# hahnicity/deepards

Measured on AMD Instinct MI355X. Metric: breath-sequences/sec (train step) cnn_linear nb20 seq224, higher is better.
Workload: dtype f32; 1 GPU; cnn_linear+resnet18, synthetic (B=64 per GPU, 20, 1, 224) fp32 train step (BASELINE configs[1]); backbone=resnet18, batch_per_gpu=64, global_batch=64, batch_rule=--batch 64 per rank (weak scaling: the global batch grows with the ranks), n_sub_batches=20, seq_len=224, optimizer=sgd-nesterov+clamp, parallelism=dp1, hipgraph=True

## Files before the change

### deepards_amd/csrc/conv_gemm.hip

```cpp
#include "common.h"
#include <algorithm>
#include <utility>
#include <vector>

#ifndef WGRAD_GLOAD_AT
#define WGRAD_GLOAD_AT 8
#endif
#ifndef GLOAD_AT
#define GLOAD_AT 3
#endif

struct ConvGemmArgs {
  const float* x;
  const float* w;
  const float* x2;
  const float* w2;
  int tap_split;
  float* y;
  int M, Lsrc, ldx, C;
  int Ldst, ldy, N;
  int dst_stride, dst_off, src_stride;
  int ntaps, so0, so1, so2, wt0, wt1, wt2;
  int accumulate;
  FastDiv divLm;
// ... 260 lines not shown
  const int lr = tid >> 3, lq = tid & 7;
  const int Lm = (int)a.divLm.d;

  const int m_a = m_blk + lr;
  const bool a_ok = m_a < a.M;
  const uint32_t row_a = fdiv((uint32_t)(a_ok ? m_a : 0), a.divLm);
  const int a_rowoff = (int)row_a * a.Lsrc;
  const int a_j = ((a_ok ? m_a : 0) - (int)row_a * Lm) * a.src_stride;

  const int kc = a.C >> 6;
  const int nk = a.ntaps * kc;
  f32x4 ra[2], rb[4];
  auto gload = [&](int it) {
    const int t = it / kc;
    const int c0 = (it - t * kc) << 6;
    const int so = t == 0 ? a.so0 : (t == 1 ? a.so1 : a.so2);
    const int wt = t == 0 ? a.wt0 : (t == 1 ? a.wt1 : a.wt2);
    const int ls = a_j + so;
    const bool ok = a_ok && ls >= 0 && ls < a.Lsrc;
    const float* src = (t < a.tap_split ? a.x : a.x2) + (size_t)(a_rowoff + (ok ? ls : 0)) * a.ldx + c0 + lq * 4;
#pragma unroll
    for (int h = 0; h < 2; ++h) {
      f32x4 v = {0.f, 0.f, 0.f, 0.f};
      if (ok) v = *reinterpret_cast<const f32x4*>(src + 32 * h);
      ra[h] = v;
    }
    const float* wtp = (t < a.tap_split ? a.w : a.w2) + (size_t)wt * a.N * a.C + c0 + lq * 4;
#pragma unroll
    for (int p = 0; p < 2; ++p)
#pragma unroll
      for (int h = 0; h < 2; ++h)
        rb[2 * p + h] = *reinterpret_cast<const f32x4*>(wtp + (size_t)(n_blk + lr + 32 * p) * a.C + 32 * h);
  };

  f32x16 acc;
#pragma unroll
  for (int r = 0; r < 16; ++r) acc[r] = 0.f;
  const int frow = lane & 31, fh = lane >> 5;
  gload(0);
  for (int it = 0; it < nk; ++it) {
    __syncthreads();
#pragma unroll
    for (int h = 0; h < 2; ++h) *reinterpret_cast<f32x4*>(&As[(h * 32 + lr) * PITCH + lq * 4]) = ra[h];
#pragma unroll
    for (int p = 0; p < 2; ++p)
#pragma unroll
      for (int h = 0; h < 2; ++h)
        *reinterpret_cast<f32x4*>(&Bs[(h * 64 + lr + 32 * p) * PITCH + lq * 4]) = rb[2 * p + h];
    __syncthreads();
#pragma unroll
    for (int c8 = 0; c8 < 4; ++c8) {
      if (c8 == 3) {
        __builtin_amdgcn_sched_barrier(0);
        if (it + 1 < nk) gload(it + 1);
        __builtin_amdgcn_sched_barrier(0);
      }
      const f32x4 af = *reinterpret_cast<const f32x4*>(&As[(ks * 32 + frow) * PITCH + c8 * 8 + fh * 4]);
      const f32x4 bf = *reinterpret_cast<const f32x4*>(&Bs[(ks * 64 + wn * 32 + frow) * PITCH + c8 * 8 + fh * 4]);
#pragma unroll
      for (int e = 0; e < 4; ++e) acc = __builtin_amdgcn_mfma_f32_32x32x2f32(af[e], bf[e], acc, 0, 0, 0);
    }
  }

  __syncthreads();
  float* red = lds;
  if (ks == 1) {
#pragma unroll
    for (int r = 0; r < 16; ++r) red[(wn * 16 + r) * 64 + lane] = acc[r];
  }
  __syncthreads();
  if (ks == 1) return;
#pragma unroll
  for (int r = 0; r < 16; ++r) acc[r] += red[(wn * 16 + r) * 64 + lane];

  size_t off[16];
  bool ok[16];
#pragma unroll
  for (int r = 0; r < 16; ++r) {
    const int m = m_blk + (r & 3) + 8 * (r >> 2) + 4 * fh;
    ok[r] = m < a.M;
    const uint32_t row = fdiv((uint32_t)(ok[r] ? m : 0), a.divLm);
    const int jj = (ok[r] ? m : 0) - (int)row * Lm;
    off[r] = ((size_t)row * a.Ldst + (size_t)(jj * a.dst_stride + a.dst_off)) * a.ldy;
  }
  const int n = n_blk + wn * 32 + frow;
  if (a.accumulate) {
    float old[16];
#pragma unroll
    for (int r = 0; r < 16; ++r) old[r] = ok[r] ? a.y[off[r] + n] : 0.f;
#pragma unroll
    for (int r = 0; r < 16; ++r)
      if (ok[r]) a.y[off[r] + n] = acc[r] + old[r];
  } else {
#pragma unroll
    for (int r = 0; r < 16; ++r)
      if (ok[r]) a.y[off[r] + n] = acc[r];
  }
}

template <bool HALO>
__global__ __launch_bounds__(256) void conv_gemm_tailed_kernel(ConvGemmArgs a, int nmini, int nmini_pad, int full) {
  __shared__ float lds[HALO ? HALO_LDS_FLOATS : TAIL_LDS_FLOATS];
  if ((int)blockIdx.x < nmini_pad) {
    if ((int)blockIdx.x < nmini) conv_tail_body(a, full + ((int)blockIdx.x >> 1), blockIdx.x & 1, lds);
    return;
  }
  if (HALO) conv3_halo_body(a, blockIdx.x - nmini_pad, full, lds);
  else conv_gemm_body<1, 1, 2, 2>(a, xcd_chunked(blockIdx.x - nmini_pad, full), lds);
}

static int g_use_tail = 1;

template <bool HALO>
static int launch_conv64(const ConvGemmArgs& a, hipStream_t s) {
  const int tiles = ((a.M + 63) / 64) * (a.N / 64);
  const int R = tiles % 256;
  if (g_use_tail && a.C % 64 == 0 && tiles > 256 && R >= 1 && R <= 128) {
    const int full = tiles - R, nmini = 2 * R, nmini_pad = (nmini + 7) / 8 * 8;
    hipLaunchKernelGGL((conv_gemm_tailed_kernel<HALO>), dim3(nmini_pad + full), dim3(256), 0, s, a, nmini, nmini_pad, full);
  } else if (HALO) {
    hipLaunchKernelGGL(conv3_halo_kernel, dim3(tiles), dim3(256), 0, s, a);
  } else {
    hipLaunchKernelGGL((conv_gemm_kernel<1, 1, 2, 2>), dim3(tiles), dim3(256), 0, s, a);
  }
  DA_CHECK_LAUNCH();
  return DA_OK;
}

static double balance(long blocks) {
  double per = (double)blocks / 256.0;
  double mx = (double)((blocks + 255) / 256);
  return per / mx;
}

struct ConvGemmTable {
  ConvGemmArgs d[4];
  int first_block[5];
  int n;
  int tail_first;
};

__global__ __launch_bounds__(256) void conv_gemm_multi_kernel(ConvGemmTable t, int nmini, int nmini_pad) {
  __shared__ float lds[TAIL_LDS_FLOATS];
  if ((int)blockIdx.x < nmini_pad) {
    if ((int)blockIdx.x < nmini) conv_tail_body(t.d[t.n - 1], t.tail_first + ((int)blockIdx.x >> 1), blockIdx.x & 1, lds);
    return;
  }
  const int g = blockIdx.x - nmini_pad;
  int i = 0;
  while (i + 1 < t.n && g >= t.first_block[i + 1]) ++i;
  conv_gemm_body<1, 1, 2, 2>(t.d[i], xcd_chunked(g - t.first_block[i], t.first_block[i + 1] - t.first_block[i]), lds);
}

static int launch_conv_multi(const ConvGemmArgs* a, int n, hipStream_t s) {
  ConvGemmTable t;
  int tiles = 0, last = 0;
  bool tail_ok = g_use_tail != 0;
  for (int i = 0; i < n; ++i) {
    t.d[i] = a[i];
    t.first_block[i] = tiles;
    last = ((a[i].M + 63) / 64) * (a[i].N / 64);
    tiles += last;
    tail_ok = tail_ok && a[i].C % 64 == 0;
  }
  t.n = n;
  if (tiles == 0) return DA_OK;
  const int R = tiles % 256;
  int nmini = 0;
  if (tail_ok && tiles > 256 && R >= 1 && R <= 128 && R < last) nmini = 2 * R;
  t.first_block[n] = tiles - nmini / 2;
  t.tail_first = last - nmini / 2;
  const int nmini_pad = (nmini + 7) / 8 * 8;
  hipLaunchKernelGGL(conv_gemm_multi_kernel, dim3(nmini_pad + t.first_block[n]), dim3(256), 0, s, t, nmini, nmini_pad);
  DA_CHECK_LAUNCH();
  return DA_OK;
}

static int conv_gemm_dispatch(const ConvGemmArgs& a, hipStream_t s) {
  if (a.M <= 0) return DA_OK;
  if (a.C % 32 || a.N % 32 || a.ldx % 4 || a.ntaps < 1 || a.ntaps > 3) return DA_EINVAL;
  if ((uint64_t)a.M * (uint64_t)a.divLm.d >= 0xffffffffull) return DA_EINVAL;
  if (a.C >= 128 && a.ntaps == 3 && a.src_stride == 1 && a.dst_stride == 1 && a.dst_off == 0 && a.N % 64 == 0 &&
      a.Lsrc == (int)a.divLm.d && a.Ldst == (int)a.divLm.d && a.so0 >= -1 && a.so0 <= 1 && a.so1 >= -1 && a.so1 <= 1 &&
      a.so2 >= -1 && a.so2 <= 1) {
    return launch_conv64<true>(a, s);
  }
  struct Cand { int id, bm, bn; double eff; };
  static const Cand cands[] = {{1, 128, 128, 1.00}, {2, 64, 128, 0.99}, {3, 128, 64, 0.97}, {4, 64, 64, 0.93},
                               {5, 128, 32, 0.85}, {6, 32, 128, 0.85}};
  int best = 0;
  double best_score = -1.0;
  for (const Cand& c : cands) {
    if (a.N % c.bn) continue;
    long blocks = (long)((a.M + c.bm - 1) / c.bm) * (a.N / c.bn);
    double score = c.eff * balance(blocks);
    if (score > best_score) {
      best_score = score;
      best = c.id;
    }
  }
  switch (best) {
    case 1: return launch_conv_gemm<2, 2, 2, 2>(a, s);
    case 2: return launch_conv_gemm<1, 2, 2, 2>(a, s);
    case 3: return launch_conv_gemm<1, 2, 4, 1>(a, s);
    case 4: return launch_conv64<false>(a, s);
    case 5: return launch_conv_gemm<1, 1, 4, 1>(a, s);
    case 6: return launch_conv_gemm<1, 1, 1, 4>(a, s);
    default: return DA_EINVAL;
  }
}

struct Conv1x1BnArgs {
  const float* x;
  const float* w;
  float* y;
  int M, ldx, C, ldy, N, W, Wn, ldstat;
  float* mean;
  float* invstd;
  const float* gamma;
  const float* beta;
  FastDiv divWn;
  const float* pend;
  int pend_c0, pend_nc, pend_Wu, pend_tiles;
  float eps;
  float* out_part;
};

template <int POOL, int OSTATS = 0>
__global__ __launch_bounds__(256) void conv1x1_bn_kernel(Conv1x1BnArgs a) {
  extern __shared__ __attribute__((aligned(16))) float lds[];
  constexpr int PITCH = 36;
  float* As = lds;
  float* Bs = lds + 64 * PITCH;
  float* scs = lds + 128 * PITCH;
  float* shs = scs + 2 * a.C;
  const int tid = threadIdx.x, lane = tid & 63, wave = tid >> 6;
  const int wm = wave >> 1, wn = wave & 1;
  const int ntn = a.N >> 6;
  const int lin = xcd_chunked(blockIdx.x, gridDim.x);
  const int m_blk = (lin / ntn) * 64, n_blk = (lin % ntn) * 64;
  const int lr = tid >> 3, lq = tid & 7;
  const int w0 = (int)fdiv((uint32_t)m_blk, a.divWn);

  int a_off[2], a_ws[2];
  bool a_ok[2];
#pragma unroll
  for (int p = 0; p < 2; ++p) {
    const int m = m_blk + lr + 32 * p;
    a_ok[p] = m < a.M;
    const int mm = a_ok[p] ? m : 0;
    a_ws[p] = ((int)fdiv((uint32_t)mm, a.divWn) - w0) * a.C + lq * 4;
    a_off[p] = (POOL ? 2 * mm : mm) * a.ldx + lq * 4;
  }
  const float* wb = a.w + (size_t)(n_blk + lr) * a.C + lq * 4;

  const int kc = a.C >> 5;
  f32x4 ra[2][POOL + 1], rb[2];
  auto gload = [&](int it) {
    const int c0 = it << 5;
#pragma unroll
    for (int p = 0; p < 2; ++p)
#pragma unroll
      for (int h = 0; h <= POOL; ++h) {
        f32x4 v = {0.f, 0.f, 0.f, 0.f};
        if (a_ok[p]) v = *reinterpret_cast<const f32x4*>(a.x + a_off[p] + h * a.ldx + c0);
        ra[p][h] = v;
      }
#pragma unroll
    for (int p = 0; p < 2; ++p) rb[p] = *reinterpret_cast<const f32x4*>(wb + (size_t)(32 * p) * a.C + c0);
  };

  f32x16 acc;
#pragma unroll
  for (int r = 0; r < 16; ++r) acc[r] = 0.f;
  gload(0);
  for (int i = tid; i < 2 * a.C; i += 256) {
    const int ws = i >= a.C ? 1 : 0, c = i - ws * a.C, w = w0 + ws;
    float sc = 0.f, sh = 0.f;
    if (w < a.W) {
      float mu, is;
      if (c >= a.pend_c0) {
        merge_stat_records(a.pend, a.pend_tiles, a.pend_nc, a.pend_Wu, w, c - a.pend_c0, a.eps, mu, is);
        const int mw = w * a.Wn;
        if (n_blk == 0 && mw >= m_blk && mw < m_blk + 64) {
          a.mean[(size_t)w * a.ldstat + c] = mu;
          a.invstd[(size_t)w * a.ldstat + c] = is;
        }
      } else {
        mu = a.mean[(size_t)w * a.ldstat + c];
        is = a.invstd[(size_t)w * a.ldstat + c];
      }
      bn_scale_shift(mu, is, a.gamma[c], a.beta[c], sc, sh);
    }
    scs[i] = sc;
    shs[i] = sh;
  }
  const int frow = lane & 31, fh = lane >> 5;
  for (int it = 0; it < kc; ++it) {
    __syncthreads();
    const int c0 = it << 5;
#pragma unroll
    for (int p = 0; p < 2; ++p) {
      const f32x4 sc = *reinterpret_cast<const f32x4*>(&scs[a_ws[p] + c0]);
      const f32x4 sh = *reinterpret_cast<const f32x4*>(&shs[a_ws[p] + c0]);
      f32x4 h;
#pragma unroll
      for (int e = 0; e < 4; ++e) {
// ... 444 lines not shown
}


static void wgrad_fill_args(WgradArgs& a, const da_wgrad_job& j, const WgradPlan& pl) {
  a.dy = j.dy; a.x = j.x; a.slab = j.workspace;
  a.M = j.rows * j.Lm; a.Ldy = j.Ldy; a.lddy = j.lddy; a.N = j.N;
  a.Lx = j.Lx; a.ldx = j.ldx; a.C = j.C;
  a.dy_stride = j.dy_stride; a.dy_off = j.dy_off; a.src_stride = j.src_stride;
  a.ntaps = j.ntaps;
  a.so0 = j.src_off[0]; a.so1 = j.ntaps > 1 ? j.src_off[1] : 0; a.so2 = j.ntaps > 2 ? j.src_off[2] : 0;
  a.kchunk = pl.kchunk;
  a.divLm = make_fastdiv((uint32_t)j.Lm);
  a.xform = j.xform; a.dy_half = j.dy_half; a.ldstat = j.ldstat;
  a.kind = 0;
  a.mean = j.mean; a.invstd = j.invstd; a.gamma = j.gamma; a.beta = j.beta;
  a.divWn = make_fastdiv((uint32_t)(j.Wn > 0 ? j.Wn : 1));
}

template <int TM, int TN, int WGM, int WGN, int XF = 0>
static int launch_wgrad_group(const da_wgrad_job* jobs, const WgradPlan* plan, int n, int tn, int tc, hipStream_t s, WgradChain* chain) {
  constexpr int BM = TM * WGM * 32, BN = TN * WGN * 32;
  WgradTable t;
  int cnt = 0, blocks = 0;
  auto flush = [&]() -> int {
    if (!cnt) return DA_OK;
    t.n = cnt;
    t.first_block[cnt] = blocks;
    WgradPreTable pre = wgrad_chain_take(chain);
    hipLaunchKernelGGL((conv_wgrad_multi_kernel<TM, TN, WGM, WGN, XF>), dim3(wgrad_pre_grid(pre, blocks, true)), dim3(256), 0, s, t, pre);
    DA_CHECK_LAUNCH();
    cnt = 0;
    blocks = 0;
    return DA_OK;
  };
  std::vector<std::pair<int, int>> order;
  for (int i = 0; i < n; ++i) {
    if (jobs[i].winograd) continue;
    if ((XF != 0) != (jobs[i].xform != 0 || jobs[i].dy_half != 0)) continue;
    if (plan[i].tn == tn && plan[i].tc == tc) order.push_back({-plan[i].kchunk, i});
  }
  std::stable_sort(order.begin(), order.end());
  for (const auto& o : order) {
    const da_wgrad_job& j = jobs[o.second];
    const WgradPlan& pl = plan[o.second];
    wgrad_fill_args(t.d[cnt], j, pl);
    t.first_block[cnt] = blocks;
    blocks += (j.N / BM) * (j.C / BN) * j.ntaps * pl.splits;
    wgrad_chain_offer(chain, o.second, j, pl.splits);
    if (++cnt == WGRAD_TABLE_MAX) {
      int rc = flush();
      if (rc) return rc;
    }
  }
  return flush();
}

static int g_wgrad_any = 1;

template <int XF>
static int launch_wgrad_any(const da_wgrad_job* jobs, const WgradPlan* plan, int n, hipStream_t s, WgradChain* chain) {
  WgradAnyTable t;
  int cnt = 0, blocks = 0;
  auto flush = [&]() -> int {
    if (!cnt) return DA_OK;
    t.n = cnt;
    t.first_block[cnt] = blocks;
    WgradPreTable pre = wgrad_chain_take(chain);
    hipLaunchKernelGGL((conv_wgrad_any_kernel<XF>), dim3(wgrad_pre_grid(pre, blocks, true)), dim3(256), 0, s, t, pre);
    DA_CHECK_LAUNCH();
    cnt = 0;
    blocks = 0;
    return DA_OK;
  };
  std::vector<std::pair<long, int>> order;
  for (int i = 0; i < n; ++i) {
    if (jobs[i].winograd) continue;
    if ((XF != 0) != (jobs[i].xform != 0 || jobs[i].dy_half != 0)) continue;
    const WgradPlan& pl = plan[i];
    if (pl.tn == 128 && pl.tc == 128) continue;
    order.push_back({-(long)pl.kchunk * (pl.tn * pl.tc / 4096), i});
  }
  std::stable_sort(order.begin(), order.end());
  for (const auto& o : order) {
    const da_wgrad_job& j = jobs[o.second];
    const WgradPlan& pl = plan[o.second];
    wgrad_fill_args(t.d[cnt], j, pl);
    t.d[cnt].kind = pl.tn == 128 ? (pl.tc == 64 ? 0 : 3) : (pl.tn == 64 ? (pl.tc == 128 ? 1 : 2) : 4);
    t.first_block[cnt] = blocks;
    blocks += (j.N / pl.tn) * (j.C / pl.tc) * j.ntaps * pl.splits;
    wgrad_chain_offer(chain, o.second, j, pl.splits);
    if (++cnt == WGRAD_TABLE_MAX) {
      int rc = flush();
      if (rc) return rc;
    }
  }
  return flush();
}

int wgrad_plan_jobs(const da_wgrad_job* jobs, int n, int chained, WgradPlan* plan) {
  if (n < 0 || (n && (!jobs || !plan))) return DA_EINVAL;
  int n_xf = 0;
  for (int i = 0; i < n; ++i) {
    const da_wgrad_job& j = jobs[i];
    if (!j.dy || !j.x || j.ntaps < 1 || j.ntaps > 3 || j.C % 32 || j.N % 32 || j.lddy % 4 || j.ldx % 4 ||
        (j.winograd == 49 && (j.lddy != j.N || j.ldx != j.C)))
      return DA_EINVAL;
    if ((uint64_t)j.rows * j.Lm * (uint64_t)j.Lm >= 0xffffffffull) return DA_EINVAL;
    if (j.winograd != 0 && j.winograd != 1 && j.winograd != 6 && j.winograd != 16 && j.winograd != 49) return DA_EINVAL;
    if ((j.xform || j.dy_half) && (j.winograd || j.src_stride != 1 || j.dy_stride != 1 || j.dy_off || j.Lm != j.Lx ||
                                   (j.dy_half && j.ntaps != 1)))
      return DA_EINVAL;
    if (j.dy_half && !j.xform) return DA_EINVAL;
    if (j.xform && (j.xform != 1 || !j.mean || !j.invstd || !j.gamma || !j.beta || j.Wn < 1 || j.ldstat < j.C || j.ldstat % 4 ||
                    j.Wn < 32 || (uint64_t)j.rows * j.Lm * (uint64_t)j.Wn >= 0xffffffffull))
      return DA_EINVAL;
    if (j.dy_half && (j.Lm & 1 || j.Ldy * 2 != j.Lm)) return DA_EINVAL;
    if (g_act_bf16 && j.winograd != 16) return DA_EINVAL;
    if (j.winograd == 16 || j.winograd == 49 ? !bf16_wgrad_eligible(j) : (j.winograd && !wino_wgrad_eligible(j))) return DA_EINVAL;
    n_xf += (j.xform || j.dy_half) ? 1 : 0;
  }
  const int tgt = (chained && g_wgrad_any && n_xf >= 8) ? (2560 / n_xf < 96 ? 96 : 2560 / n_xf) : 0;
  for (int i = 0; i < n; ++i) {
    const da_wgrad_job& j = jobs[i];
    plan[i].tn = plan[i].tc = 64;
    if (j.winograd == 16 || j.winograd == 49) bf16_wgrad_plan(j.rows, j.Lm, &plan[i].splits, &plan[i].kchunk);
    else if (j.winograd == 6) wino4_wgrad_plan(j.rows, j.Lm, &plan[i].splits, &plan[i].kchunk);
    else if (j.winograd == 0) {
      plan[i] = wgrad_plan(j.rows * j.Lm, j.N, j.C, j.ntaps, (j.xform || j.dy_half) ? tgt : 0);
      if (!plan[i].tn) return DA_EINVAL;
    }
  }
  wino_wgrad_plan_jobs(jobs, n, chained, plan);
  return DA_OK;
}

static void conv_gemm_fill(ConvGemmArgs& g, const da_conv_job& j) {
  g.x = j.x; g.w = j.w; g.y = j.y;
  g.x2 = j.x2 ? j.x2 : j.x; g.w2 = j.w2 ? j.w2 : j.w; g.tap_split = j.x2 ? j.tap_split : 3;
  g.M = j.rows * j.Lm; g.Lsrc = j.Lsrc; g.ldx = j.ldx; g.C = j.C;
  g.Ldst = j.Ldst; g.ldy = j.ldy; g.N = j.N;
  g.dst_stride = j.dst_stride; g.dst_off = j.dst_off; g.src_stride = j.src_stride;
  g.ntaps = j.ntaps;
  g.so0 = j.src_off[0]; g.so1 = j.ntaps > 1 ? j.src_off[1] : 0; g.so2 = j.ntaps > 2 ? j.src_off[2] : 0;
  g.wt0 = j.wtap[0]; g.wt1 = j.ntaps > 1 ? j.wtap[1] : 0; g.wt2 = j.ntaps > 2 ? j.wtap[2] : 0;
  g.accumulate = j.accumulate;
  g.divLm = make_fastdiv((uint32_t)j.Lm);
}

extern "C" {

int da_debug_set(int key, int value) {
  if (key == 3) g_use_tail = value;
  else if (key == 7) g_wgrad_any = value;
  else return DA_EINVAL;
  return DA_OK;
}

int da_conv_gemm(const float* x, const float* w, float* y, int rows, int Lm, int Lsrc, int ldx, int C, int Ldst,
                 int ldy, int N, int dst_stride, int dst_off, int src_stride, int ntaps, const int* src_off,
                 const int* wtap, int accumulate, hipStream_t stream) {
  DA_ENTER();
  if (g_act_bf16) return DA_EINVAL;
  if (!x || !w || !y || rows < 0 || Lm < 1 || ntaps < 1 || ntaps > 3) return DA_EINVAL;
  da_conv_job j = {};
  j.x = x; j.w = w; j.y = y;
  j.rows = rows; j.Lm = Lm; j.Lsrc = Lsrc; j.ldx = ldx; j.C = C; j.Ldst = Ldst; j.ldy = ldy; j.N = N;
  j.dst_stride = dst_stride; j.dst_off = dst_off; j.src_stride = src_stride; j.ntaps = ntaps; j.accumulate = accumulate;
  for (int t = 0; t < ntaps; ++t) {
    j.src_off[t] = src_off[t];
    j.wtap[t] = wtap[t];
  }
  ConvGemmArgs a;
  conv_gemm_fill(a, j);
  return conv_gemm_dispatch(a, stream);
}

int da_conv_gemm_multi(const da_conv_job* jobs, int n, hipStream_t stream) {
  DA_ENTER();
  if (g_act_bf16) return DA_EINVAL;
  if (n < 1 || n > 4 || !jobs) return DA_EINVAL;
  ConvGemmArgs a[4];
  for (int i = 0; i < n; ++i) {
    const da_conv_job& j = jobs[i];
    if (!j.x || !j.w || !j.y || j.rows < 0 || j.Lm < 1 || j.ntaps < 1 || j.ntaps > 3 || j.C % 32 || j.N % 64 || j.ldx % 4)
      return DA_EINVAL;
    if ((uint64_t)j.rows * j.Lm * (uint64_t)j.Lm >= 0xffffffffull) return DA_EINVAL;
    if (j.x2 && (!j.w2 || j.tap_split < 1 || j.tap_split >= j.ntaps)) return DA_EINVAL;
    conv_gemm_fill(a[i], j);
  }
  return launch_conv_multi(a, n, stream);
}

int da_conv1x1_bn(const float* x, int ldx, const float* w, float* y, int ldy, int rows, int R, int Lin, int C, int N, int pool,
                  float* mean, float* invstd, int ldstat, const float* gamma, const float* beta, const float* pend, int pend_c0,
                  long pend_units, int pend_Wu, float eps, float* out_part, hipStream_t stream) {
  DA_ENTER();
  if (g_act_bf16) return DA_EINVAL;
  if (!x || !w || !y || !mean || !invstd || !gamma || !beta || rows < 0 || R < 1 || rows % R || Lin < 1) return DA_EINVAL;
  if (C % 32 || C < 32 || C > 2048 || N % 64 || N < 64 || ldx % 4 || ldx < C || ldy < N || ldstat % 4 || ldstat < C) return DA_EINVAL;
  if (pool && (Lin & 1)) return DA_EINVAL;
  if (rows == 0) return DA_OK;
  const int Lout = pool ? Lin / 2 : Lin;
  const long M = (long)rows * Lout;
  if ((long)R * Lout < 64) return DA_EINVAL;
  if ((uint64_t)rows * Lin * (uint64_t)(ldx > ldy ? ldx : ldy) >= 0x7fffffffull) return DA_EINVAL;
  if ((uint64_t)M * (uint64_t)(R * Lout) >= 0xffffffffull) return DA_EINVAL;
  Conv1x1BnArgs a;
  a.x = x; a.w = w; a.y = y;
  a.M = (int)M; a.ldx = ldx; a.C = C; a.ldy = ldy; a.N = N; a.W = rows / R; a.Wn = R * Lout; a.ldstat = ldstat;
  a.mean = mean; a.invstd = invstd; a.gamma = gamma; a.beta = beta;
  a.divWn = make_fastdiv((uint32_t)a.Wn);
  a.pend = pend; a.pend_c0 = C; a.pend_nc = 0; a.pend_Wu = 1; a.pend_tiles = 0; a.eps = eps; a.out_part = out_part;
  if (pend) {
    if (pend_c0 < 0 || pend_c0 >= C || pend_units < 1 || pend_Wu < 64 || pend_units % pend_Wu || pend_units / pend_Wu != rows / R)
      return DA_EINVAL;
    a.pend_c0 = pend_c0; a.pend_nc = C - pend_c0; a.pend_Wu = pend_Wu; a.pend_tiles = (int)((pend_units + 63) / 64);
  }
  const unsigned blocks = (unsigned)(((M + 63) / 64) * (N / 64));
  const size_t shm = (size_t)(128 * 36 + 4 * C) * sizeof(float);
  if (out_part) {
    if (pool) hipLaunchKernelGGL((conv1x1_bn_kernel<1, 1>), dim3(blocks), dim3(256), shm, stream, a);
    else hipLaunchKernelGGL((conv1x1_bn_kernel<0, 1>), dim3(blocks), dim3(256), shm, stream, a);
  } else if (pool) hipLaunchKernelGGL((conv1x1_bn_kernel<1, 0>), dim3(blocks), dim3(256), shm, stream, a);
  else hipLaunchKernelGGL((conv1x1_bn_kernel<0, 0>), dim3(blocks), dim3(256), shm, stream, a);
  DA_CHECK_LAUNCH();
  return DA_OK;
}

size_t da_conv_wgrad_workspace(int rows, int Lm, int N, int C, int ntaps) {
  WgradPlan p = wgrad_plan(rows * Lm, N, C, ntaps);
  return (size_t)p.splits * ntaps * N * C * sizeof(float);
}

static int conv_wgrad_multi_impl(const da_wgrad_job* jobs, int n, int chained, float* const* dws, int accumulate, int* reduced,
                                 hipStream_t stream) {
  DA_ENTER();
  std::vector<WgradPlan> plan_(n > 0 ? n : 0);
  WgradPlan* const plan = plan_.data();
  int rc = wgrad_plan_jobs(jobs, n, chained, plan);
  if (rc) return rc;
  for (int i = 0; i < n; ++i)
    if (!jobs[i].workspace) return DA_EINVAL;
  WgradChain chain_, *chain = nullptr;
  if (dws) {
    if (!reduced) return DA_EINVAL;
    for (int i = 0; i < n; ++i) reduced[i] = 0;
    wgrad_chain_init(&chain_, dws, accumulate, reduced);
    chain = &chain_;
  }
  if ((rc = wino4_wgrad_launch(jobs, plan, n, stream, chain))) return rc;
  if ((rc = wino_wgrad_launch(jobs, plan, n, stream, chain))) return rc;
  if ((rc = bf16_wgrad_launch(jobs, plan, n, 49, stream))) return rc;
  if ((rc = bf16_wgrad_launch(jobs, plan, n, 16, stream))) return rc;
  if ((rc = launch_wgrad_group<2, 2, 2, 2>(jobs, plan, n, 128, 128, stream, chain))) return rc;
  if ((rc = launch_wgrad_group<2, 1, 2, 2>(jobs, plan, n, 128, 64, stream, chain))) return rc;
  if ((rc = launch_wgrad_group<1, 2, 2, 2>(jobs, plan, n, 64, 128, stream, chain))) return rc;
  if ((rc = launch_wgrad_group<1, 1, 2, 2>(jobs, plan, n, 64, 64, stream, chain))) return rc;
  if ((rc = launch_wgrad_group<1, 1, 4, 1>(jobs, plan, n, 128, 32, stream, chain))) return rc;
  if ((rc = launch_wgrad_group<1, 1, 1, 4>(jobs, plan, n, 32, 128, stream, chain))) return rc;
  if ((rc = launch_wgrad_group<2, 2, 2, 2, 1>(jobs, plan, n, 128, 128, stream, chain))) return rc;
  if (g_wgrad_any) return launch_wgrad_any<1>(jobs, plan, n, stream, chain);
  if ((rc = launch_wgrad_group<2, 1, 2, 2, 1>(jobs, plan, n, 128, 64, stream, chain))) return rc;
  if ((rc = launch_wgrad_group<1, 2, 2, 2, 1>(jobs, plan, n, 64, 128, stream, chain))) return rc;
  if ((rc = launch_wgrad_group<1, 1, 2, 2, 1>(jobs, plan, n, 64, 64, stream, chain))) return rc;
  if ((rc = launch_wgrad_group<1, 1, 4, 1, 1>(jobs, plan, n, 128, 32, stream, chain))) return rc;
  return launch_wgrad_group<1, 1, 1, 4, 1>(jobs, plan, n, 32, 128, stream, chain);
}

int da_conv_wgrad_multi(const da_wgrad_job* jobs, int n, hipStream_t stream) {
  return conv_wgrad_multi_impl(jobs, n, 0, nullptr, 0, nullptr, stream);
}

int da_conv_wgrad_multi_reduce(const da_wgrad_job* jobs, int n, float* const* dws, int accumulate, int* reduced,
                               hipStream_t stream) {
  if (n && (!dws || !reduced)) return DA_EINVAL;
  return conv_wgrad_multi_impl(jobs, n, 1, dws, accumulate, reduced, stream);
}

int da_conv_wgrad_plan(const da_wgrad_job* jobs, int n, int chained, int* slabs) {
  if (n > 0 && !slabs) return DA_EINVAL;
  std::vector<WgradPlan> plan(n > 0 ? n : 0);
  const int rc = wgrad_plan_jobs(jobs, n, chained, plan.data());
  for (int i = 0; !rc && i < n; ++i) slabs[i] = plan[i].splits;
  return rc;
}

int da_conv_wgrad_splits(int rows, int Lm, int N, int C, int ntaps) {
  return wgrad_plan(rows * Lm, N, C, ntaps).splits;
}

typedef struct {
  const float* slab;
  float* dw;
  int splits, ntaps, N, C;
} da_wgrad_reduce_desc;

int da_sizeof_wgrad_reduce_desc(void) { return (int)sizeof(da_wgrad_reduce_desc); }

typedef struct {
  const float* s1;
  const float* s2;
  float* dgamma;
  float* dbeta;
  int W, C;
} da_bn_pgrad_desc;
typedef struct {
// ... 126 lines not shown
```

Baseline: 453,600 breath-sequences/s.

## Fuse paired strided conv and shortcut GEMMs into one kernel sharing input tiles

Adds a pair kernel for the case where a grouped conv launch holds two jobs reading the same input. This covers a stride-2 3-tap conv plus a 1x1 downsample in the forward pass, and a matching pair in dgrad. Each block loads the shared input tile into LDS once and computes both outputs with two MFMA accumulators, instead of running separate tile sets that reload the input. The cost is a larger LDS footprint and occupancy capped at 3 blocks per CU, plus specialised pattern matching that can fall back to the old multi-job kernel.

```diff
diff --git a/deepards_amd/csrc/conv_gemm.hip b/deepards_amd/csrc/conv_gemm.hip
--- a/deepards_amd/csrc/conv_gemm.hip
+++ b/deepards_amd/csrc/conv_gemm.hip
@@ -436,7 +436,199 @@
   conv_gemm_body<1, 1, 2, 2>(t.d[i], xcd_chunked(g - t.first_block[i], t.first_block[i + 1] - t.first_block[i]), lds);
 }
 
+#define PAIR_LDS_FLOATS ((65 + 64 + 4 * 64) * 32)
+static_assert(PAIR_LDS_FLOATS >= TAIL_LDS_FLOATS, "the half tiles of a pair launch use the pair's LDS");
+
+__device__ __forceinline__ void conv_store_tile32(const ConvGemmArgs& a, const f32x16& acc, const int m0, const int n, const int fh) {
+  const int Lm = (int)a.divLm.d;
+  size_t off[16];
+  bool ok[16];
+#pragma unroll
+  for (int r = 0; r < 16; ++r) {
+    const int m = m0 + (r & 3) + 8 * (r >> 2) + 4 * fh;
+    ok[r] = m < a.M;
+    const uint32_t row = fdiv((uint32_t)(ok[r] ? m : 0), a.divLm);
+    const int jj = (ok[r] ? m : 0) - (int)row * Lm;
+    off[r] = ((size_t)row * a.Ldst + (size_t)(jj * a.dst_stride + a.dst_off)) * a.ldy;
+  }
+  if (a.accumulate) {
+    float old[16];
+#pragma unroll
+    for (int r = 0; r < 16; ++r) old[r] = ok[r] ? a.y[off[r] + n] : 0.f;
+#pragma unroll
+    for (int r = 0; r < 16; ++r)
+      if (ok[r]) a.y[off[r] + n] = acc[r] + old[r];
+  } else {
+#pragma unroll
+    for (int r = 0; r < 16; ++r)
+      if (ok[r]) a.y[off[r] + n] = acc[r];
+  }
+}
+
+template <bool DGRAD>
+__device__ __forceinline__ void conv_pair_body(const ConvGemmArgs& p, const ConvGemmArgs& q, const int lin, float* lds) {
+  constexpr int BN = 64, R_P0 = 0, R_P1 = 65, R_B = 65 + 64;
+  auto at = [&](int row, int slot) { return lds + row * 32 + ((slot ^ (row >> 1)) & 7) * 4; };
+
+  const int tid = threadIdx.x, lane = tid & 63, wave = tid >> 6;
+  const int wm = wave >> 1, wn = wave & 1;
+  const int ntn = p.N / BN;
+  const int m_blk = (lin / ntn) * 64, n_blk = (lin % ntn) * BN;
+  const int lr = tid >> 3, lq = tid & 7;
+  const int Lm = (int)p.divLm.d;
+  const int kc = p.C >> 5;
+  const size_t nc = (size_t)p.N * p.C;
+
+  const float* x0 = p.x;
+  const float* x1 = DGRAD ? q.x2 : p.x;
+  const float* wB[4];
+  wB[0] = p.w + p.wt0 * nc;
+  wB[1] = p.w + p.wt1 * nc;
+  wB[2] = DGRAD ? q.w + q.wt0 * nc : p.w + p.wt2 * nc;
+  wB[3] = DGRAD ? q.w2 + q.wt1 * nc : q.w + q.wt0 * nc;
+
+  const int npos = DGRAD ? p.M : 2 * p.M;
+  int pos[5];
+  bool pok[5];
+#pragma unroll
+  for (int i = 0; i < 5; ++i) {
+    const int e = i < 4 ? lr + 32 * (i & 1) : 64;
+    const bool odd_plane = i < 2 || i == 4;
+    pos[i] = DGRAD ? m_blk + e : 2 * (m_blk + e) - (odd_plane ? 1 : 0);
+    pok[i] = pos[i] >= 0 && pos[i] < npos && (i < 4 || tid < 8);
+  }
+
+  f32x4 ra[5], rb[8];
+  auto gload = [&](int ks) {
+    const int c0 = (ks << 5) + lq * 4;
+#pragma unroll
+    for (int i = 0; i < 5; ++i) {
+      const float* src = (i < 2 || i == 4 ? x0 : x1) + (size_t)(pok[i] ? pos[i] : 0) * p.ldx + c0;
+      f32x4 v = {0.f, 0.f, 0.f, 0.f};
+      if (pok[i]) v = *reinterpret_cast<const f32x4*>(src);
+      ra[i] = v;
+    }
+#pragma unroll
+    for (int i = 0; i < 8; ++i)
+      rb[i] = *reinterpret_cast<const f32x4*>(wB[i >> 1] + (size_t)(n_blk + lr + 32 * (i & 1)) * p.C + c0);
+  };
+
+  const int frow = lane & 31, fh = lane >> 5;
+  const int m_lane = m_blk + wm * 32 + frow;
+  const uint32_t rowq = fdiv((uint32_t)(m_lane < p.M ? m_lane : 0), p.divLm);
+  const int j_lane = (m_lane < p.M ? m_lane : 0) - (int)rowq * Lm;
+  const bool dead = DGRAD ? j_lane == Lm - 1 : j_lane == 0;
+
+  f32x16 acc0, acc1;
+#pragma unroll
+  for (int r = 0; r < 16; ++r) acc0[r] = acc1[r] = 0.f;
+
+  const int a_row0 = R_P0 + wm * 32 + frow, a_row1 = R_P1 + wm * 32 + frow, b_row = R_B + wn * 32 + frow;
+
+  gload(0);
+  for (int ks = 0; ks < kc; ++ks) {
+    __syncthreads();
+#pragma unroll
+    for (int i = 0; i < 2; ++i) *reinterpret_cast<f32x4*>(at(R_P0 + lr + 32 * i, lq)) = ra[i];
+#pragma unroll
+    for (int i = 0; i < 2; ++i) *reinterpret_cast<f32x4*>(at(R_P1 + lr + 32 * i, lq)) = ra[2 + i];
+    if (tid < 8) *reinterpret_cast<f32x4*>(at(R_P0 + 64, lq)) = ra[4];
+#pragma unroll
+    for (int i = 0; i < 8; ++i) *reinterpret_cast<f32x4*>(at(R_B + (i >> 1) * BN + lr + 32 * (i & 1), lq)) = rb[i];
+    __syncthreads();
+#pragma unroll
+    for (int t = 0; t < 4; ++t) {
+      const int ar = DGRAD ? (t == 0 ? a_row0 + 1 : (t == 3 ? a_row1 : a_row0)) : (t == 0 ? a_row0 : (t == 2 ? a_row0 + 1 : a_row1));
+      const bool second = DGRAD ? t >= 2 : t == 3;
+#pragma unroll
+      for (int c8 = 0; c8 < 4; ++c8) {
+        if (t == 3 && c8 == 1) {
+          __builtin_amdgcn_sched_barrier(0);
+          if (ks + 1 < kc) gload(ks + 1);
+          __builtin_amdgcn_sched_barrier(0);
+        }
+        f32x4 af = *reinterpret_cast<const f32x4*>(at(ar, c8 * 2 + fh));
+        const f32x4 bf = *reinterpret_cast<const f32x4*>(at(b_row + t * BN, c8 * 2 + fh));
+        if (t == 0 && dead) af = f32x4{0.f, 0.f, 0.f, 0.f};
+#pragma unroll
+        for (int e = 0; e < 4; ++e) {
+          if (second) acc1 = __builtin_amdgcn_mfma_f32_32x32x2f32(af[e], bf[e], acc1, 0, 0, 0);
+          else acc0 = __builtin_amdgcn_mfma_f32_32x32x2f32(af[e], bf[e], acc0, 0, 0, 0);
+        }
+      }
+    }
+  }
+
+  const int n = n_blk + wn * 32 + frow;
+  conv_store_tile32(p, acc0, m_blk + wm * 32, n, fh);
+  conv_store_tile32(q, acc1, m_blk + wm * 32, n, fh);
+}
+
+template <bool DGRAD>
+__device__ __forceinline__ void conv_pair_kernel_body(const ConvGemmTable& t, const int nmini, const int nmini_pad, float* lds) {
+  if ((int)blockIdx.x < nmini_pad) {
+    const int b = blockIdx.x;
+    if (b < nmini) conv_tail_body(t.d[(b >> 1) & 1], t.tail_first + (b >> 2), b & 1, lds);
+    return;
+  }
+  conv_pair_body<DGRAD>(t.d[0], t.d[1], xcd_chunked(blockIdx.x - nmini_pad, t.first_block[1]), lds);
+}
+
+__global__ __launch_bounds__(256, 3) void conv_gemm_multi_kernel_pair_fwd(ConvGemmTable t, int nmini, int nmini_pad) {
+  __shared__ float lds[PAIR_LDS_FLOATS];
+  conv_pair_kernel_body<false>(t, nmini, nmini_pad, lds);
+}
+
+__global__ __launch_bounds__(256, 3) void conv_gemm_multi_kernel_pair_dgrad(ConvGemmTable t, int nmini, int nmini_pad) {
+  __shared__ float lds[PAIR_LDS_FLOATS];
+  conv_pair_kernel_body<true>(t, nmini, nmini_pad, lds);
+}
+
+static int g_use_pair = 1;
+
+static int conv_pair_kind(const ConvGemmArgs* a, int n, int* first) {
+  if (!g_use_pair || n != 2) return 0;
+  const ConvGemmArgs &u = a[0], &v = a[1];
+  const int Lm = (int)u.divLm.d;
+  if (u.x != v.x || u.M != v.M || u.Lsrc != v.Lsrc || u.ldx != v.ldx || u.C != v.C || u.N != v.N || Lm != (int)v.divLm.d) return 0;
+  if (u.C % 64 || u.N % 64 || u.M >= (1 << 29)) return 0;
+  for (int i = 0; i < 2; ++i) {
+    const ConvGemmArgs &p = a[i], &q = a[1 - i];
+    *first = i;
+    if (p.Lsrc == 2 * Lm && p.src_stride == 2 && q.src_stride == 2 && p.ntaps == 3 && p.tap_split >= 3 && p.so0 == -1 &&
+        p.so1 == 0 && p.so2 == 1 && q.ntaps == 1 && q.so0 == 0)
+      return 1;
+    if (p.Lsrc == Lm && p.src_stride == 1 && q.src_stride == 1 && p.ntaps == 2 && p.tap_split >= 2 && p.so0 == 1 && p.so1 == 0 &&
+        q.ntaps == 2 && q.tap_split == 1 && q.so0 == 0 && q.so1 == 0)
+      return 2;
+  }
+  return 0;
+}
+
+static int launch_conv_pair(const ConvGemmArgs& p, const ConvGemmArgs& q, int kind, hipStream_t s) {
+  ConvGemmTable t;
+  t.d[0] = p;
+  t.d[1] = q;
+  t.n = 2;
+  const int tiles = ((p.M + 63) / 64) * (p.N / 64);
+  if (tiles == 0) return DA_OK;
+  const int R = tiles % 256;
+  int nmini = 0;
+  if (g_use_tail && tiles > 256 && R >= 1 && R <= 128) nmini = 4 * R;
+  t.first_block[0] = 0;
+  t.first_block[1] = t.first_block[2] = t.tail_first = tiles - nmini / 4;
+  const int nmini_pad = (nmini + 7) / 8 * 8;
+  if (kind == 1)
+    hipLaunchKernelGGL(conv_gemm_multi_kernel_pair_fwd, dim3(nmini_pad + t.first_block[1]), dim3(256), 0, s, t, nmini, nmini_pad);
+  else
+    hipLaunchKernelGGL(conv_gemm_multi_kernel_pair_dgrad, dim3(nmini_pad + t.first_block[1]), dim3(256), 0, s, t, nmini, nmini_pad);
+  DA_CHECK_LAUNCH();
+  return DA_OK;
+}
+
 static int launch_conv_multi(const ConvGemmArgs* a, int n, hipStream_t s) {
+  int first = 0;
+  if (const int kind = conv_pair_kind(a, n, &first)) return launch_conv_pair(a[first], a[1 - first], kind, s);
   ConvGemmTable t;
   int tiles = 0, last = 0;
   bool tail_ok = g_use_tail != 0;
@@ -1187,6 +1379,7 @@
 int da_debug_set(int key, int value) {
   if (key == 3) g_use_tail = value;
   else if (key == 7) g_wgrad_any = value;
+  else if (key == 9) g_use_pair = value;
   else return DA_EINVAL;
   return DA_OK;
 }
```

Result: slower. 448,700 breath-sequences/s (-1.1%).
